# jluuser/PyTorch-VAE

Hardware: AMD Instinct MI355X
Metric: train images/sec @64x64x3 bs256 (curve tensors [B,64,6], SURVEY.md s0) (higher is better)
Workload: dtype f32; 1 GPU; C2: stage2_vq.yaml model with num_quantizers=1 K=512 D=64 N=64; full train step (fwd+loss+bwd+clip+AdamW+EMA), dropout 0.1, loss weights at epoch 100; per_gpu_batch=256, global_batch=256, seq_len=64, parallelism=dp1, hipgraph=True, params=43115078

## Files before the change

### pytorch-vae_amd/csrc/gemm.hip

```cpp
#include "common.h"
#include <type_traits>
#include <utility>
#include <vector>
#include <algorithm>

namespace {

constexpr int BM = 128, BN = 128;
constexpr int BK = 32;
template <int BKT> struct Tile {
    static constexpr int KC_LD = BKT + 4;
    static constexpr int A_TILE = BM * KC_LD;
    static constexpr int NLD = BKT / 8;
};

enum EpiMode {
    EPI_LINEAR = 0,
    EPI_RELU_DROP = 1,
    EPI_GELU = 2,
    EPI_DROP_RESID = 3,
    EPI_SIGMOID = 4,
    EPI_MUL_POSMASK = 5,
    EPI_MUL_GELUGRAD = 6,
    EPI_MUL_SIGGRAD = 7,
// ... 600 lines not shown
    for (int i = threadIdx.x; i < M * nq; i += 256) {
        f32x4 v = *reinterpret_cast<const f32x4*>(red + (size_t)i * 4);
        for (int s2 = 1; s2 < slices; ++s2) v += *reinterpret_cast<const f32x4*>(red + (size_t)s2 * M * N + (size_t)i * 4);
        *reinterpret_cast<f32x4*>(out + (size_t)i * 4) = v;
    }
    if (rs && threadIdx.x < M) {
        float t = 0.f;
        for (int s2 = 0; s2 < slices; ++s2) t += red_rs[s2][threadIdx.x];
        rs[(size_t)blockIdx.x * M + threadIdx.x] = t;
    }
}

#include "gemm_dma.inc"
#include "gemm_p3.inc"

struct ProfRec { int slot; double flops; hipEvent_t e0, e1; };
bool g_prof_on = false;
std::vector<ProfRec> g_prof;
constexpr int PROF_MODES = 9;
constexpr int PROF_FAMILIES = 7;
inline int prof_slot(bool a_kc, bool b_kc, int mode_t, int family = 0) {
    return (family * 4 + (a_kc ? 2 : 0) + (b_kc ? 1 : 0)) * PROF_MODES + mode_t + 1;
}

template <bool A_KC, bool B_KC, int BKT, int MODE = -1>
int launch(const GemmArgs& g, int splits, hipStream_t stream) {
    static bool attr_set = false;
    const size_t smem = (size_t)4 * Tile<BKT>::A_TILE * sizeof(float);
    if (!attr_set) {
        hipError_t e = hipFuncSetAttribute(reinterpret_cast<const void*>(&gemm_f32_mfma<A_KC, B_KC, BKT, MODE>),
// ... 89 lines not shown
            rc = VQH_ERR_LAUNCH;
        } else if (out) {
            out[r.slot * 3 + 0] += 1.0;
            out[r.slot * 3 + 1] += (double)ms * 1e-3;
            out[r.slot * 3 + 2] += r.flops;
        }
        (void)hipEventDestroy(r.e0);
        (void)hipEventDestroy(r.e1);
    }
    g_prof.clear();
    return rc;
}

extern "C" int vqh_reduce_slabs(const float* slabs, int S, long long stride, long long n, float* out, float beta,
                                hipStream_t stream);

static int g_gemm_flags = 1;
extern "C" int vqh_gemm_set_flags(int flags) {
#ifndef VQH_DIAG
    flags &= ~(2 | 4);
#endif
    const int old = g_gemm_flags; g_gemm_flags = flags; return old;
}

static int gemm_impl(int a_kcontig, int b_kcontig, int M, int N, int K, const float* A, int lda, const float* B,
                     int ldb, float* C, int ldc, const float* bias, int mode, const float* aux_in, float* aux_out,
                     int ldaux, float beta, const unsigned long long* rng_state, unsigned drop_site, float drop_p,
                     float* workspace, long long workspace_floats, float* rowsum, hipStream_t stream) {
    VQH_CHECK_ARG(M >= 0 && N >= 0 && K >= 0, "vqh_gemm: negative dimension");
    if (M == 0 || N == 0) return VQH_OK;
// ... 195 lines not shown
extern "C" int vqh_gemm_wgrad(int rows, int n_out, int k_in, const float* dY, int lddy, const float* X, int ldx, float* dW,
                              int lddw, float* db, float beta, float* workspace, long long workspace_floats,
                              hipStream_t stream) {
    if (rows > 0 && n_out > 0 && k_in == 0) return VQH_OK;
    return gemm_impl(0, 0, n_out, k_in, rows, dY, lddy, X, ldx, dW, lddw, nullptr, EPI_LINEAR, nullptr, nullptr, 0, beta,
                     nullptr, 0, 0.f, workspace, workspace_floats, db, stream);
}

struct vqh_wgrad_t {
    int rows, n_out, k_in;
    const float* dY; int lddy;
    const float* X; int ldx;
    float* dW; int lddw;
    float* db;
};
extern "C" int vqh_gemm_wgrad_group(int n, const vqh_wgrad_t* pr, float* workspace, long long workspace_floats,
                                    hipStream_t stream) {
    VQH_CHECK_ARG(n >= 0 && (n == 0 || pr), "vqh_gemm_wgrad_group: bad argument");
    auto al16 = [](const void* q) { return (reinterpret_cast<uintptr_t>(q) & 15) == 0; };
    std::vector<int> big;
    for (int i = 0; i < n; ++i) {
        const vqh_wgrad_t& w = pr[i];
        VQH_CHECK_ARG(w.rows >= 0 && w.n_out >= 0 && w.k_in >= 0, "vqh_gemm_wgrad_group: negative dimension");
        const bool ok = !(g_gemm_flags & (128 | 256)) && workspace && w.rows >= 8 * dma::TBK && (w.rows % dma::TBK) == 0 &&
                        (w.n_out % dma::TBM) == 0 && (w.k_in % dma::TBN) == 0 && w.n_out > 0 && w.k_in > 0 && al16(w.dY) &&
                        al16(w.X) && al16(w.dW) && al16(workspace) && (w.lddy & 3) == 0 && (w.ldx & 3) == 0 && (w.lddw & 3) == 0 &&
                        w.lddy >= w.n_out && w.ldx >= w.k_in && w.lddw >= w.k_in;
        if (ok) {
            big.push_back(i);
        } else {
            const int rc = vqh_gemm_wgrad(w.rows, w.n_out, w.k_in, w.dY, w.lddy, w.X, w.ldx, w.dW, w.lddw, w.db, 0.f, workspace,
                                          workspace_floats, stream);
            if (rc != VQH_OK) return rc;
        }
    }
    for (size_t c0 = 0; c0 < big.size(); c0 += GROUP_MAX) {
        const int m = (int)std::min<size_t>(GROUP_MAX, big.size() - c0);
        long long tiles_tot = 0;
        int kmax = 0;
        for (int j = 0; j < m; ++j) {
            const vqh_wgrad_t& w = pr[big[c0 + j]];
            tiles_tot += (long long)(w.n_out / dma::TBM) * (w.k_in / dma::TBN);
            kmax = std::max(kmax, w.rows);
        }
        int best_kc = kmax;
        double best = -1.0;
        for (int sp = 1; sp <= 64; ++sp) {
            const int kc = ((kmax + sp - 1) / sp + dma::TBK - 1) / dma::TBK * dma::TBK;
            if (kc < 16 * dma::TBK && sp > 1) break;
            long long wgs = 0, slab = 0;
            for (int j = 0; j < m; ++j) {
                const vqh_wgrad_t& w = pr[big[c0 + j]];
                const int splits = (w.rows + kc - 1) / kc;
                wgs += (long long)(w.n_out / dma::TBM) * (w.k_in / dma::TBN) * splits;
                if (splits > 1) slab += (long long)splits * ((long long)w.n_out * w.k_in + w.n_out);
            }
            if (slab > workspace_floats) continue;
            const double rounds = (double)((wgs + 255) / 256);
// ... 27 lines not shown
                off += (long long)splits * w.n_out * w.k_in;
                g.rowsum_ws = w.db ? workspace + off : nullptr;
                if (w.db) off += (long long)splits * w.n_out;
                off = (off + 3) / 4 * 4;
                red[nred++] = Red{g.ws, splits, w.n_out, w.k_in, w.dW, w.lddw, g.rowsum_ws, w.db};
            } else {
                g.ws = nullptr;
                g.rowsum_ws = nullptr;
            }
            G.tiles[j] = (w.n_out / dma::TBM) * (w.k_in / dma::TBN);
            G.wg_begin[j] = wg;
            wg += G.tiles[j] * splits;
            flops += 2.0 * w.n_out * (double)w.k_in * w.rows;
        }
        for (int j = m; j <= GROUP_MAX; ++j) G.wg_begin[j] = wg;
        static bool attr_set = false;
        if (!attr_set) {
            hipError_t e = hipFuncSetAttribute(reinterpret_cast<const void*>(&gemm_f32_dma_group),
                                               hipFuncAttributeMaxDynamicSharedMemorySize, dma::LDS_BYTES);
            if (e == hipSuccess)
                e = hipFuncSetAttribute(reinterpret_cast<const void*>(&gemm_f32_x3_group), hipFuncAttributeMaxDynamicSharedMemorySize,
                                        dma::LDS_BYTES);
            if (e != hipSuccess) { vqh_set_error(hipGetErrorString(e)); return VQH_ERR_LAUNCH; }
            attr_set = true;
        }
        const bool native = (g_gemm_flags & 512) != 0;
        ProfRec rec{};
        if (g_prof_on) {
            rec.slot = prof_slot(false, false, EPI_LINEAR, native ? 2 : 4);
            rec.flops = flops;
            if (hipEventCreate(&rec.e0) != hipSuccess || hipEventCreate(&rec.e1) != hipSuccess ||
                hipEventRecord(rec.e0, stream) != hipSuccess) {
                vqh_set_error("vqh_gemm_wgrad_group: profiling events failed");
                return VQH_ERR_LAUNCH;
            }
        }
        if (native) hipLaunchKernelGGL(gemm_f32_dma_group, dim3(wg), dim3(256), dma::LDS_BYTES, stream, G);
        else hipLaunchKernelGGL(gemm_f32_x3_group, dim3(wg), dim3(256), dma::LDS_BYTES, stream, G);
        VQH_LAUNCH_CHECK();
        if (g_prof_on) {
            if (hipEventRecord(rec.e1, stream) != hipSuccess) {
// ... 55 lines not shown
            VQH_CHECK_ARG(it.X && it.P && it.rows > 0 && it.cols > 0 && (it.cols % 32) == 0 && it.ldx >= it.cols && (it.ldx & 3) == 0 &&
                          it.pitch_bytes >= (long long)it.cols * 6 && (it.pitch_bytes % 16) == 0 &&
                          ((reinterpret_cast<uintptr_t>(it.X) | reinterpret_cast<uintptr_t>(it.P)) & 15) == 0,
                          "vqh_p3_split_multi: bad item (cols % 32, alignment, pitch)");
            S.it[i] = P3SplitItem{it.X, reinterpret_cast<char*>(it.P), it.rows, it.cols, it.ldx, it.pitch_bytes};
            most = std::max(most, (long long)it.rows * (it.cols >> 3));
        }
        int bx = (int)std::min<long long>((most + 255) / 256, 512);
        hipLaunchKernelGGL(p3_split_multi_kernel, dim3(bx, S.n), dim3(256), 0, stream, S);
        VQH_LAUNCH_CHECK();
    }
    return VQH_OK;
}

namespace {
inline int p3_num_cus() {
    static int n = 0;
    if (n == 0) {
        int dev = 0;
        hipDeviceProp_t prop;
        if (hipGetDevice(&dev) == hipSuccess && hipGetDeviceProperties(&prop, dev) == hipSuccess && prop.multiProcessorCount > 0)
            n = prop.multiProcessorCount;
        else n = 256;
    }
    return n;
}
template <bool A_KC, bool B_KC, int MODE>
int launch_p3(const P3Args& g, int splits, hipStream_t stream) {
    static bool attr_set = false;
    auto kern = &gemm_p3<A_KC, B_KC, MODE>;
    if (!attr_set) {
        hipError_t e = hipFuncSetAttribute(reinterpret_cast<const void*>(kern), hipFuncAttributeMaxDynamicSharedMemorySize, p3::LDS_BYTES);
        if (e != hipSuccess) { vqh_set_error(hipGetErrorString(e)); return VQH_ERR_LAUNCH; }
        attr_set = true;
    }
    const int n_items = (g.M / p3::TBM) * (g.N / p3::TBN) * splits;
    dim3 grid(std::min(n_items, p3_num_cus()));
    if (((g.kchunk / p3::TBK) & 1) && n_items > (int)grid.x) grid.x = n_items;
    ProfRec rec{};
    if (g_prof_on) {
        rec.slot = prof_slot(A_KC, B_KC, MODE, 5);
// ... 275 lines not shown
```

### pytorch-vae_amd/csrc/gemm_dma.inc

```

namespace dma {
constexpr int TBM = 256, TBN = 128, TBK = 32;
constexpr int A_BYTES = TBM * TBK * 4, B_BYTES = TBN * TBK * 4, STAGE_BYTES = A_BYTES + B_BYTES;
constexpr int NSTAGE = 3, LDS_BYTES = NSTAGE * STAGE_BYTES;
constexpr int DMA_A = A_BYTES / 1024 / 4, DMA_B = B_BYTES / 1024 / 4, DMA_PER_WAVE = DMA_A + DMA_B;
constexpr int MI = 4, NJ = 2;
}

typedef float f32x2 __attribute__((ext_vector_type(2)));

typedef unsigned u32x2 __attribute__((ext_vector_type(2)));
typedef unsigned u32x4 __attribute__((ext_vector_type(4)));
typedef short s16x4 __attribute__((ext_vector_type(4)));
typedef __bf16 bf16x8 __attribute__((ext_vector_type(8)));

namespace x3 {
constexpr int A_PLANE = dma::TBM * dma::TBK * 2, B_PLANE = dma::TBN * dma::TBK * 2;
constexpr int B_OFF = 3 * A_PLANE;
constexpr int STAGE_BYTES = 3 * (A_PLANE + B_PLANE);
constexpr int LDS_BYTES = 2 * STAGE_BYTES;
constexpr int NU = 12, NUA = 8;
constexpr int NB = 8, G = 48, NSLOT = 96;
constexpr int BAR = 7 * NU;
constexpr int RS_OFF = 40960;
// ... 34 lines not shown
    __device__ __forceinline__ void all(const f32x4& a) { step<0>(a); step<1>(a); step<2>(a); step<3>(a); step<4>(a); }
};

__device__ __forceinline__ void glds16_s(const char* ubase, unsigned voff, unsigned lds_byte_addr_uniform) {
    asm volatile("s_mov_b32 m0, %2\n\ts_nop 0\n\tglobal_load_lds_dwordx4 %0, %1"
                 :
                 : "v"(voff), "s"(ubase), "s"(lds_byte_addr_uniform)
                 : "memory");
}

__device__ __forceinline__ void glds16(const float* gptr, unsigned lds_byte_addr_uniform) {
    __builtin_amdgcn_global_load_lds(gptr, (__attribute__((address_space(3))) void*)(uintptr_t)lds_byte_addr_uniform, 16, 0, 0);
}

template <bool A_KC, bool B_KC, int MODE, bool X3 = false>
__device__ __forceinline__ void gemm_dma_tile(const GemmArgs& g, const int tile, const int zsplit) {
    using namespace dma;
    constexpr bool EA_KC = X3 ? true : A_KC, EB_KC = X3 ? true : B_KC;
    extern __shared__ __attribute__((aligned(1024))) unsigned char smem_dma[];
    const int tid = threadIdx.x, lane = tid & 63;
    const int wave = __builtin_amdgcn_readfirstlane(tid >> 6);
    const int wm = wave >> 1, wn = wave & 1;
    const int l31 = lane & 31, h = lane >> 5;

    const int tiles_n = g.N / TBN;
    const int m0 = (tile / tiles_n) * TBM, n0 = (tile % tiles_n) * TBN;
    const int kbeg = zsplit * g.kchunk;
    const int kend = min(g.K, kbeg + g.kchunk);
    const int nk = (kend - kbeg) / TBK;

    unsigned voff[DMA_PER_WAVE];
    unsigned dst[DMA_PER_WAVE];
#pragma unroll
    for (int i = 0; i < DMA_A; ++i) {
        const int j = wave + 4 * i;
        if (A_KC) {
            const int R = j * 8 + (lane >> 3), c = (lane & 7) ^ ((R >> 1) & 7);
            voff[i] = (unsigned)(((size_t)R * g.lda + c * 4) * 4);
        } else {
            voff[i] = (unsigned)(((size_t)j * g.lda + lane * 4) * 4);
        }
        dst[i] = j * 1024;
    }
// ... 215 lines not shown
                return *reinterpret_cast<const u32x4*>(sb + x3::B_OFF + pl * x3::B_PLANE + j * 2048 + rB[gg]);
            } else {
                const unsigned a0 = (unsigned)(uintptr_t)(sb + x3::B_OFF + pl * x3::B_PLANE + (16 * gg) * 256 + rB[j]);
                const s16x4 lo = __builtin_amdgcn_ds_read_tr16_b64_v4i16((__attribute__((address_space(3))) s16x4*)(uintptr_t)a0);
                const s16x4 hi = __builtin_amdgcn_ds_read_tr16_b64_v4i16((__attribute__((address_space(3))) s16x4*)(uintptr_t)(a0 + 4 * 256));
                const u32x2 l2 = __builtin_bit_cast(u32x2, lo), h2 = __builtin_bit_cast(u32x2, hi);
                return u32x4{l2[0], l2[1], h2[0], h2[1]};
            }
        };
        auto aux_one = [&](auto q_c) {
            constexpr int q = decltype(q_c)::value;
            auxr[q] = *reinterpret_cast<const f32x4*>(g.aux_in + (size_t)(m0 + wm * 128 + (lane >> 4) + q * 4) * g.ldaux + col);
        };
        if (nk > 0) {
            static_for<x3::NU>([&](auto u_c) { load_unit(u_c, 0); });
            if (HAS_DROP && g.drop.p > 0.f && !g.ws) {
#pragma unroll
                for (int qi = 0; qi < 32; ++qi) hash_quad(qi);
            }
            static_for<x3::NU>([&](auto u_c) {
                constexpr int u = decltype(u_c)::value;
                if (do_rowsum && u < x3::NUA) {
#pragma unroll
                    for (int e = 0; e < 4; ++e) rs[e] += st[u][e];
                }
                su.all(st[u]);
                write_unit(u_c, I0{}, smem_dma);
                write_unit(u_c, I1{}, smem_dma);
                write_unit(u_c, I2{}, smem_dma);
                load_unit(u_c, nk > 1 ? 1 : 0);
            });
            asm volatile("s_waitcnt lgkmcnt(0)" ::: "memory");
            __builtin_amdgcn_s_barrier();
            static_for<4>([&](auto i_c) { xA[0][decltype(i_c)::value] = read_A(I0{}, i_c, I0{}, smem_dma); });
            static_for<6>([&](auto x_c) {
                constexpr int x = decltype(x_c)::value;
                xB[0][x / 2][x % 2] = read_B(std::integral_constant<int, x / 2>{}, std::integral_constant<int, x % 2>{}, I0{}, smem_dma);
            });
            auto kstep = [&](auto last_c, const int kt) {
                constexpr bool LAST = decltype(last_c)::value;
                const unsigned char* rstg = smem_dma + (kt & 1) * x3::STAGE_BYTES;
                unsigned char* wstg = smem_dma + ((kt & 1) ^ 1) * x3::STAGE_BYTES;
                const int kt_ld = min(kt + 2, nk - 1);
                const bool want_aux = LAST && HAS_AUX && !g.ws;
                static_for<x3::NSLOT>([&](auto m_c) {
                    constexpr int m = decltype(m_c)::value;
                    constexpr int gg = m / x3::G, mm = m % x3::G, pi = mm / x3::NB, b = mm % x3::NB, i = b / 2, j = b % 2;
                    constexpr int pa = (pi < 3) ? 0 : (pi < 5) ? 1 : 2;
                    constexpr int pb = (pi == 0 || pi == 3 || pi == 5) ? 0 : (pi == 1 || pi == 4) ? 1 : 2;
                    acc[i][j] = __builtin_amdgcn_mfma_f32_32x32x16_bf16(__builtin_bit_cast(bf16x8, xA[pa][i]),
                                                                        __builtin_bit_cast(bf16x8, xB[gg][pb][j]), acc[i][j], 0, 0, 0);
                    if constexpr (m < 8 && m % 2 == 0) xA[1][m / 2] = read_A(I1{}, std::integral_constant<int, m / 2>{}, I0{}, rstg);
                    if constexpr (m >= 8 && m < 16 && m % 2 == 0) xA[2][(m - 8) / 2] = read_A(I2{}, std::integral_constant<int, (m - 8) / 2>{}, I0{}, rstg);
                    if constexpr (m >= 16 && m < 28 && m % 2 == 0) {
                        constexpr int x = (m - 16) / 2;
                        xB[1][x / 2][x % 2] = read_B(std::integral_constant<int, x / 2>{}, std::integral_constant<int, x % 2>{}, I1{}, rstg);
                    }
                    if constexpr (m >= 28 && m < 44 && m % 4 == 0) xA[0][(m - 28) / 4] = read_A(I0{}, std::integral_constant<int, (m - 28) / 4>{}, I1{}, rstg);
                    if constexpr (m >= 48 && m < 56 && m % 2 == 0) xA[1][(m - 48) / 2] = read_A(I1{}, std::integral_constant<int, (m - 48) / 2>{}, I1{}, rstg);
// ... 24 lines not shown
                        if constexpr (m == x3::BAR - 1) {
                            asm volatile("s_waitcnt lgkmcnt(0)" ::: "memory");
                            __builtin_amdgcn_s_barrier();
                        }
                    } else if constexpr (HAS_AUX) {
                        if constexpr (m % 3 == 0) {
                            if (want_aux) aux_one(std::integral_constant<int, m / 3>{});
                        }
                    }
                    __builtin_amdgcn_sched_barrier(0);
                });
            };
            for (int kt = 0; kt < nk - 1; ++kt) kstep(std::false_type{}, kt);
            kstep(std::true_type{}, nk - 1);
            __builtin_amdgcn_s_barrier();
        } else if (HAS_AUX && !g.ws) {
            load_aux_all();
        }
    } else
    if (nk > 0) {
        issue_all(0, 0);
        issue_all(nk > 1 ? 1 : 0, 1);
        if (HAS_DROP && g.drop.p > 0.f && !g.ws) {
#pragma unroll
            for (int qi = 0; qi < 32; ++qi) hash_quad(qi);
        }
        asm volatile("s_waitcnt vmcnt(%0)" ::"n"(DMA_PER_WAVE) : "memory");
        __builtin_amdgcn_s_barrier();
        read_first(0);
        int stage = 0;
        for (int kt = 0; kt < nk; ++kt) {
            const int nxt = (stage == 2) ? 0 : stage + 1;
            const int nx2 = (nxt == 2) ? 0 : nxt + 1;
            if (HAS_AUX && !g.ws && kt == nk - 1) load_aux_all();
            substep(I0{}, I1{}, I0{}, I0{}, stage, 0, 0);
            substep(I1{}, I2{}, I0{}, I0{}, stage, 0, 0);
            asm volatile("s_waitcnt vmcnt(0)" ::: "memory");
            __builtin_amdgcn_s_barrier();
            const int ktd = min(kt + 2, nk - 1);
            substep(I0{}, I3{}, I0{}, IH{}, stage, ktd, nx2);
            substep(I1{}, I0{}, IH{}, IF{}, nxt, ktd, nx2);
            stage = nxt;
        }
        asm volatile("s_waitcnt vmcnt(0)" ::: "memory");
        __builtin_amdgcn_s_barrier();
    } else if (HAS_AUX && !g.ws) {
        load_aux_all();
    }

    if (X3 && do_rowsum) {
        float* rsb = reinterpret_cast<float*>(smem_dma + x3::RS_OFF);
        *reinterpret_cast<f32x4*>(rsb + wave * TBM + 4 * lane) = f32x4{rs[0], rs[1], rs[2], rs[3]};
        __builtin_amdgcn_s_barrier();
        if (wave == 0) {
            f32x4 t = *reinterpret_cast<const f32x4*>(rsb + 4 * lane);
#pragma unroll
            for (int w = 1; w < 4; ++w) t += *reinterpret_cast<const f32x4*>(rsb + w * TBM + 4 * lane);
            const int row = m0 + 4 * lane;
            if (g.rowsum_ws) {
                *reinterpret_cast<f32x4*>(g.rowsum_ws + (size_t)zsplit * g.M + row) = t;
            } else {
#pragma unroll
                for (int i = 0; i < 4; ++i) g.rowsum[row + i] = (g.beta != 0.f) ? g.beta * g.rowsum[row + i] + t[i] : t[i];
            }
        }
    } else
    if (do_rowsum) {
#pragma unroll
        for (int i = 0; i < 4; ++i) rs[i] += __shfl_xor(rs[i], 32, 64);
        if (h == 0) {
            const int row = m0 + wm * 128 + 4 * l31;
            if (g.rowsum_ws) {
                *reinterpret_cast<f32x4*>(g.rowsum_ws + (size_t)zsplit * g.M + row) = f32x4{rs[0], rs[1], rs[2], rs[3]};
            } else {
#pragma unroll
                for (int i = 0; i < 4; ++i)
                    g.rowsum[row + i] = (g.beta != 0.f) ? g.beta * g.rowsum[row + i] + rs[i] : rs[i];
            }
        }
    }

    const int mode = (MODE >= 0) ? MODE : g.mode;
    constexpr int EP_LD = 68;
    float* ep = reinterpret_cast<float*>(smem_dma) + wave * (32 * EP_LD);
    float* slab = g.ws ? g.ws + (size_t)zsplit * g.M * g.N : nullptr;
    if constexpr (X3 && MODE == EPI_LINEAR) {
        if (!(g.flags & 2048)) {
            const size_t ldo = slab ? (size_t)g.N : (size_t)g.ldc;
            float* obase = slab ? slab : g.C;
#pragma unroll
            for (int j = 0; j < NJ; ++j) {
                const int cj = n0 + wn * 64 + j * 32 + l31;
                const float bj = (g.bias && !slab) ? g.bias[cj] : 0.f;
                float* cp = obase + (size_t)(m0 + wm * 128 + 4 * h) * ldo + cj;
                if (!slab && g.beta != 0.f) {
#pragma unroll
                    for (int i = 0; i < MI; ++i)
#pragma unroll
                        for (int r = 0; r < 16; ++r) {
                            float* q = cp + (size_t)(i * 32 + (r & 3) + 8 * (r >> 2)) * ldo;
// ... 74 lines not shown
                } else if (mode == EPI_MUL_GELUGRAD) {
#pragma unroll
                    for (int e = 0; e < 4; ++e) v[e] *= gelu_erf_grad(a[e]);
                } else {
#pragma unroll
                    for (int e = 0; e < 4; ++e) v[e] *= a[e] * (1.f - a[e]);
                }
            }
            if (g.beta != 0.f) v += g.beta * *reinterpret_cast<const f32x4*>(cptr);
            *reinterpret_cast<f32x4*>(cptr) = v;
        }
        __builtin_amdgcn_s_waitcnt(0xC07F);
    }
}

template <bool A_KC, bool B_KC, int MODE>
__global__ __launch_bounds__(256, 1) void gemm_f32_dma(const GemmArgs g) {
    const int nx = gridDim.x, nt = nx * gridDim.z, lin = blockIdx.z * nx + blockIdx.x;
    const int q = nt >> 3, r = nt & 7, x = lin & 7, j = lin >> 3;
    const int v = (x < r ? x * (q + 1) : r * (q + 1) + (x - r) * q) + j;
    gemm_dma_tile<A_KC, B_KC, MODE>(g, v % nx, v / nx);
}

template <bool A_KC, bool B_KC, int MODE>
__global__ __launch_bounds__(256, 1) void gemm_f32_x3(const GemmArgs g) {
    const int nx = gridDim.x, nt = nx * gridDim.z, lin = blockIdx.z * nx + blockIdx.x;
    const int q = nt >> 3, r = nt & 7, x = lin & 7, j = lin >> 3;
    const int v = (x < r ? x * (q + 1) : r * (q + 1) + (x - r) * q) + j;
    gemm_dma_tile<A_KC, B_KC, MODE, true>(g, v % nx, v / nx);
}
// ... 16 lines not shown
    const int v = ((G.p[0].flags & 1) && !(G.p[0].flags & 1024)) ? group_logical_id() : (int)blockIdx.x;
    int p = 0;
    while (p + 1 < G.n && v >= G.wg_begin[p + 1]) ++p;
    const int local = v - G.wg_begin[p];
    const int tiles = G.tiles[p];
    gemm_dma_tile<false, false, EPI_LINEAR>(G.p[p], local % tiles, local / tiles);
}
__global__ __launch_bounds__(256, 1) void gemm_f32_x3_group(const GemmGroupArgs G) {
    const int v = ((G.p[0].flags & 1) && !(G.p[0].flags & 1024)) ? group_logical_id() : (int)blockIdx.x;
    int p = 0;
    while (p + 1 < G.n && v >= G.wg_begin[p + 1]) ++p;
    const int local = v - G.wg_begin[p];
    const int tiles = G.tiles[p];
    gemm_dma_tile<false, false, EPI_LINEAR, true>(G.p[p], local % tiles, local / tiles);
}
```

### pytorch-vae_amd/csrc/loss.hip

```cpp
#include "common.h"

namespace {

enum { T_VALID = 0, T_PAIR = 1, T_TRI = 2, T_QUAD = 3, T_FIVE = 4, T_ANY3 = 5, T_PDM = 8, T_LR = 40 };

enum {
    P_RAW = 0, P_ALN, P_BEST, P_RMSD_RAW, P_RMSD_BEST, P_CE, P_ACC, P_SSTV, P_BL, P_BA, P_DIR, P_DIH, P_TV2, P_TAU,
    P_PDM, P_LRPDM, P_WINK, P_COMMIT, P_KAPPA, P_COUNT
};

enum {
    M_LOSS = 0, M_REC_XYZ, M_MSE_RAW, M_MSE_ALN, M_REC_SS, M_SS_ACC, M_VQ_LOSS, M_BL, M_BA, M_DIR, M_DIH, M_GEOM,
    M_SS_TV, M_USAGE_REG, M_TV2, M_PPL, M_DEAD, M_RMSD_RAW, M_RMSD_ALN, M_PDM, M_WINK, M_KAPPA, M_TAU, M_LRPDM, M_COUNT
};

struct LossCfg {
    int B, L, Ntok, D;
    int Ls;
    const float* Ldev;
    int masked;
    int use_vq;
    float rmsd_w, ss_w, bl_w, ba_w, dir_w, dih_w, tv_l, pdm_w, wk_w, kap_w, tau_w, lr_w;
    float alpha, ss_tv_l, label_smoothing, beta;
    int pdm_window, wk_size, wk_stride, lr_sep, lr_stride, lr_max;
// ... 205 lines not shown
        double R[9];
        kabsch_rotation(Hm, R);
        bool ok = true;
        for (int k = 0; k < 9; ++k) { Rt_s[k] = (float)R[k]; ok = ok && isfinite(R[k]); }
        for (int j = 0; j < 3; ++j) {
            const double t = bmu[j] - (amu[0] * R[0 * 3 + j] + amu[1] * R[1 * 3 + j] + amu[2] * R[2 * 3 + j]);
            Rt_s[9 + j] = (float)t;
            ok = ok && isfinite(t);
        }
        Rt_s[12] = ok ? 1.f : 0.f;
    }
    __syncthreads();
    return Rt_s[12] != 0.f;
}

__global__ __launch_bounds__(256) void loss_counts_kernel(const unsigned char* __restrict__ mask, LossCfg c_in,
                                                          int* __restrict__ table) {
    const LossCfg c = loss_resolve(c_in);
    extern __shared__ unsigned char sm_[];
    unsigned char* m = sm_;
    const int b = blockIdx.x, L = c.L;
    for (int l = threadIdx.x; l < L; l += 256) m[l] = mask ? mask[(size_t)b * c.Ls + l] : 1;
    __syncthreads();
    int nv = 0, np = 0, nt = 0, nq = 0, n5 = 0;
    for (int l = threadIdx.x; l < L; l += 256) {
        nv += m[l];
        if (l + 1 < L) np += m[l] & m[l + 1];
        if (l + 2 < L) nt += m[l] & m[l + 1] & m[l + 2];
        if (l + 3 < L) nq += m[l] & m[l + 1] & m[l + 2] & m[l + 3];
        if (l + 4 < L) n5 += m[l] & m[l + 1] & m[l + 2] & m[l + 3] & m[l + 4];
    }
    __shared__ int red[5];
    if (threadIdx.x < 5) red[threadIdx.x] = 0;
    __syncthreads();
    atomicAdd(&red[0], nv); atomicAdd(&red[1], np); atomicAdd(&red[2], nt); atomicAdd(&red[3], nq); atomicAdd(&red[4], n5);
    __syncthreads();
    if (threadIdx.x == 0) {
        atomicAdd(&table[T_VALID], red[0]); atomicAdd(&table[T_PAIR], red[1]); atomicAdd(&table[T_TRI], red[2]);
        atomicAdd(&table[T_QUAD], red[3]); atomicAdd(&table[T_FIVE], red[4]);
        if (red[0] >= 3) atomicAdd(&table[T_ANY3], 1);
    }
    for (int d = 1 + (threadIdx.x >> 6); d < c.pdm_window && d < 32; d += 4) {
        int s = 0;
        for (int l = threadIdx.x & 63; l + d < L; l += 64) s += m[l] & m[l + d];
        for (int o = 32; o > 0; o >>= 1) s += __shfl_xor(s, o, 64);
        if ((threadIdx.x & 63) == 0 && s) atomicAdd(&table[T_PDM + d - 1], s);
    }
    {
        int p = 0;
        for (int off = 0; off < max(1, c.lr_max); ++off)
            for (int i = 0; i < L; i += max(1, c.lr_stride)) {
                const int j = i + c.lr_sep + off;
                if (j >= L) break;
                if ((p & 255) == (int)threadIdx.x && (m[i] & m[j])) atomicAdd(&table[T_LR + p], 1);
                ++p;
            }
    }
    for (int w = threadIdx.x; w < c.n_windows; w += 256) {
        const int s0 = w * max(1, c.wk_stride);
        int cnt = 0;
        for (int l = 0; l < c.wk_size; ++l) cnt += m[s0 + l];
        if (!c.masked || cnt >= 3) atomicAdd(&table[c.t_wk + w], 1);
    }
}

#define FOR_POS(n_) for (int base_ = 0; base_ < (n_); base_ += 256)

__global__ __launch_bounds__(256) void loss_sample_kernel(const float* __restrict__ recons,
                                                          const float* __restrict__ target,
                                                          const unsigned char* __restrict__ mask,
                                                          const float* __restrict__ ze, const float* __restrict__ zq,
                                                          const int* __restrict__ table, LossCfg c_in,
                                                          float* __restrict__ d_recons, float* __restrict__ d_ze,
                                                          float* __restrict__ part) {
    extern __shared__ __attribute__((aligned(16))) float sm[];
    const LossCfg c = loss_resolve(c_in);
    const int L = c.L, b = blockIdx.x, tid = threadIdx.x;
    double* dred = reinterpret_cast<double*>(sm);
// ... 461 lines not shown
    for (int k = 0; k < 3; ++k) { c.sd[k] = data_stats ? data_stats[k] : 1.f; c.mu[k] = data_stats ? data_stats[3 + k] : 0.f; }
    VQH_CHECK_ARG(c.pdm_window <= 33, "vqh_loss_fwd_bwd: pdm_window > 33 unsupported");
    int npairs = 0, nwin = 0;
    loss_enumerate(L_dev ? L_stride : L, c.lr_sep, c.lr_stride, c.lr_max, c.wk_size, c.wk_stride, &npairs, &nwin);
    c.n_lr_pairs = npairs;
    c.n_windows = nwin;
    c.t_wk = T_LR + npairs;
    const long long table_ints = c.t_wk + nwin + 8;
    const long long need = table_ints + (long long)B * P_COUNT;
    VQH_CHECK_ARG(need <= workspace_floats, "vqh_loss_fwd_bwd: workspace too small");
    int* table = reinterpret_cast<int*>(workspace);
    float* part = workspace + table_ints;
    hipError_t e = hipMemsetAsync(table, 0, sizeof(int) * table_ints, stream);
    if (e != hipSuccess) { vqh_set_error(hipGetErrorString(e)); return VQH_ERR_LAUNCH; }
    const int Lmax = c.L;
    hipLaunchKernelGGL(loss_counts_kernel, dim3(B), dim3(256), (size_t)Lmax, stream, mask, c, table);
    const size_t smem = sizeof(float) * (size_t)(8 + 23 * Lmax + 4 + 16 + 9 * Lmax + 4);
    VQH_CHECK_ARG(smem <= 160 * 1024, "vqh_loss_fwd_bwd: sequence too long for the LDS-resident loss kernel");
    static bool attr_set = false;
    if (!attr_set) {
        hipError_t ea = hipFuncSetAttribute(reinterpret_cast<const void*>(&loss_sample_kernel),
                                            hipFuncAttributeMaxDynamicSharedMemorySize, 160 * 1024);
        if (ea != hipSuccess) { vqh_set_error(hipGetErrorString(ea)); return VQH_ERR_LAUNCH; }
        attr_set = true;
    }
    hipLaunchKernelGGL(loss_sample_kernel, dim3(B), dim3(256), smem, stream, recons, target, mask, ze, zq, table, c,
                       d_recons, d_ze, part);
    hipLaunchKernelGGL(loss_finish_kernel, dim3(1), dim3(64), 0, stream, part, table, c, vq_stats, metrics);
    VQH_LAUNCH_CHECK();
    return VQH_OK;
}
// ... 1 lines not shown
```

Before: 9684 images/s.

## Balance grouped wgrad GEMM via stream-K ranges and batch loss count kernel

```diff
diff --git a/pytorch-vae_amd/csrc/gemm.hip b/pytorch-vae_amd/csrc/gemm.hip
--- a/pytorch-vae_amd/csrc/gemm.hip
+++ b/pytorch-vae_amd/csrc/gemm.hip
@@ -638,6 +638,49 @@
 #include "gemm_dma.inc"
 #include "gemm_p3.inc"
 
+struct RedRangeArgs {
+    GroupRangePlan P;
+    struct Item { const float* ws; int M, N; float* C; int ldc; const float* rs_ws; float* rowsum; } r[GROUP_MAX];
+};
+__global__ __launch_bounds__(256) void splitk_reduce_ranges(const RedRangeArgs G) {
+    const GroupRangePlan& P = G.P;
+    const int gt = blockIdx.y;
+    int p = 0;
+    while (p + 1 < P.n && gt >= P.tbeg[p + 1]) ++p;
+    const int tile = gt - P.tbeg[p], nk = P.nk[p];
+    const int t0 = P.sbeg[p] + tile * nk, t1 = t0 + nk;
+    int v = min(P.wgs - 1, (int)(((long long)t0 * P.wgs) / P.total));
+    while (range_bound(P, v + 1) <= t0) ++v;
+    while (range_bound(P, v) > t0) --v;
+    int cnt = 1;
+    while (range_bound(P, v + cnt) < t1) ++cnt;
+    if (cnt == 1) return;
+    const RedRangeArgs::Item& it = G.r[p];
+    const int tiles_n = it.N / dma::TBN;
+    const int m0 = (tile / tiles_n) * dma::TBM, n0 = (tile % tiles_n) * dma::TBN;
+    const int tid = threadIdx.x;
+    if (it.rowsum && n0 == 0 && blockIdx.x == 0) {
+        float s = 0.f;
+        for (int z = 0; z < cnt; ++z) s += it.rs_ws[(size_t)z * it.M + m0 + tid];
+        it.rowsum[m0 + tid] = s;
+    }
+    const size_t total = (size_t)it.M * it.N;
+    const int row0 = m0 + 64 * blockIdx.x + (tid >> 5), col = n0 + (tid & 31) * 4;
+    const float* src = it.ws + (size_t)row0 * it.N + col;
+    f32x4 s[8];
+#pragma unroll
+    for (int i = 0; i < 8; ++i) s[i] = f32x4{0.f, 0.f, 0.f, 0.f};
+    for (int z = 0; z < cnt; ++z) {
+        f32x4 x[8];
+#pragma unroll
+        for (int i = 0; i < 8; ++i) x[i] = *reinterpret_cast<const f32x4*>(src + (size_t)z * total + (size_t)(8 * i) * it.N);
+#pragma unroll
+        for (int i = 0; i < 8; ++i) s[i] += x[i];
+    }
+#pragma unroll
+    for (int i = 0; i < 8; ++i) *reinterpret_cast<f32x4*>(it.C + (size_t)(row0 + 8 * i) * it.ldc + col) = s[i];
+}
+
 struct ProfRec { int slot; double flops; hipEvent_t e0, e1; };
 bool g_prof_on = false;
 std::vector<ProfRec> g_prof;
@@ -757,6 +800,18 @@
 
 extern "C" int vqh_reduce_slabs(const float* slabs, int S, long long stride, long long n, float* out, float beta,
                                 hipStream_t stream);
+
+static int gemm_num_cus() {
+    static int n = 0;
+    if (n == 0) {
+        int dev = 0;
+        hipDeviceProp_t prop;
+        if (hipGetDevice(&dev) == hipSuccess && hipGetDeviceProperties(&prop, dev) == hipSuccess && prop.multiProcessorCount > 0)
+            n = prop.multiProcessorCount;
+        else n = 256;
+    }
+    return n;
+}
 
 static int g_gemm_flags = 1;
 extern "C" int vqh_gemm_set_flags(int flags) {
@@ -982,6 +1037,95 @@
     float* dW; int lddw;
     float* db;
 };
+constexpr int VQH_DEFER = -1000;
+static int wgrad_group_ranges(int m, const vqh_wgrad_t* pr, const int* sel, float* workspace, long long workspace_floats,
+                              bool native, hipStream_t stream) {
+    GroupRangePlan P;
+    P.n = m; P.wgs = gemm_num_cus(); P.snap = 2;
+    long long tot = 0;
+    int tiles_tot = 0;
+    for (int j = 0; j < m; ++j) {
+        const vqh_wgrad_t& w = pr[sel[j]];
+        const int tiles = (w.n_out / dma::TBM) * (w.k_in / dma::TBN);
+        P.nk[j] = w.rows / dma::TBK;
+        P.sbeg[j] = (int)tot; P.tbeg[j] = tiles_tot;
+        tot += (long long)tiles * P.nk[j];
+        tiles_tot += tiles;
+        if (tot >= (1LL << 30) || tiles_tot > 65535) return VQH_DEFER;
+    }
+    for (int j = m; j <= GROUP_MAX; ++j) { P.sbeg[j] = (int)tot; P.tbeg[j] = tiles_tot; }
+    for (int j = m; j < GROUP_MAX; ++j) P.nk[j] = 1;
+    P.total = (int)tot; P.q = P.total / P.wgs; P.r = P.total % P.wgs;
+    if (P.q < 16 || P.wgs > 32768) return VQH_DEFER;
+    std::vector<int> cuts(tiles_tot, 0);
+    for (int v = 1; v < P.wgs; ++v) {
+        const int b = range_bound(P, v), p = range_problem(P, b), local = b - P.sbeg[p];
+        if (local % P.nk[p]) ++cuts[P.tbeg[p] + local / P.nk[p]];
+    }
+    GemmGroupArgs G;
+    RedRangeArgs RG;
+    G.n = m;
+    RG.P = P;
+    long long off = 0;
+    double flops = 0.0;
+    bool any = false;
+    for (int j = 0; j < m; ++j) {
+        const vqh_wgrad_t& w = pr[sel[j]];
+        int slabs = 1;
+        for (int t = P.tbeg[j]; t < P.tbeg[j + 1]; ++t) slabs = std::max(slabs, 1 + cuts[t]);
+        GemmArgs& g = G.p[j];
+        g.A = w.dY; g.B = w.X; g.C = w.dW;
+        g.M = w.n_out; g.N = w.k_in; g.K = w.rows;
+        g.lda = w.lddy; g.ldb = w.ldx; g.ldc = w.lddw;
+        g.kchunk = w.rows;
+        g.vecA = g.vecB = g.vecC = 1;
+        g.mode = EPI_LINEAR; g.bias = nullptr; g.aux_in = nullptr; g.aux_out = nullptr; g.ldaux = 0; g.beta = 0.f;
+        g.drop = make_drop(nullptr, 0, 0.f);
+        g.flags = g_gemm_flags;
+        g.rowsum = w.db;
+        g.ws = nullptr; g.rowsum_ws = nullptr;
+        if (slabs > 1) {
+            g.ws = workspace + off;
+            off += (long long)slabs * w.n_out * w.k_in;
+            if (w.db) { g.rowsum_ws = workspace + off; off += (long long)slabs * w.n_out; }
+            off = (off + 3) / 4 * 4;
+            any = true;
+        }
+        RG.r[j] = RedRangeArgs::Item{g.ws, w.n_out, w.k_in, w.dW, w.lddw, g.rowsum_ws, w.db};
+        G.tiles[j] = P.tbeg[j + 1] - P.tbeg[j];
+        G.wg_begin[j] = 0;
+        flops += 2.0 * w.n_out * (double)w.k_in * w.rows;
+    }
+    for (int j = m; j <= GROUP_MAX; ++j) G.wg_begin[j] = 0;
+    for (int j = m; j < GROUP_MAX; ++j) { G.tiles[j] = 0; RG.r[j] = RedRangeArgs::Item{nullptr, 0, 0, nullptr, 0, nullptr, nullptr}; }
+    if (off > workspace_floats) return VQH_DEFER;
+    ProfRec rec{};
+    if (g_prof_on) {
+        rec.slot = prof_slot(false, false, EPI_LINEAR, native ? 2 : 4);
+        rec.flops = flops;
+        if (hipEventCreate(&rec.e0) != hipSuccess || hipEventCreate(&rec.e1) != hipSuccess ||
+            hipEventRecord(rec.e0, stream) != hipSuccess) {
+            vqh_set_error("vqh_gemm_wgrad_group: profiling events failed");
+            return VQH_ERR_LAUNCH;
+        }
+    }
+    if (native) hipLaunchKernelGGL(gemm_f32_dma_group_ranges, dim3(P.wgs), dim3(256), dma::LDS_BYTES, stream, G, P);
+    else hipLaunchKernelGGL(gemm_f32_x3_group_ranges, dim3(P.wgs), dim3(256), dma::LDS_BYTES, stream, G, P);
+    VQH_LAUNCH_CHECK();
+    if (g_prof_on) {
+        if (hipEventRecord(rec.e1, stream) != hipSuccess) {
+            vqh_set_error("vqh_gemm_wgrad_group: profiling events failed");
+            return VQH_ERR_LAUNCH;
+        }
+        g_prof.push_back(rec);
+    }
+    if (any) {
+        hipLaunchKernelGGL(splitk_reduce_ranges, dim3(4, tiles_tot), dim3(256), 0, stream, RG);
+        VQH_LAUNCH_CHECK();
+    }
+    return VQH_OK;
+}
+
 extern "C" int vqh_gemm_wgrad_group(int n, const vqh_wgrad_t* pr, float* workspace, long long workspace_floats,
                                     hipStream_t stream) {
     VQH_CHECK_ARG(n >= 0 && (n == 0 || pr), "vqh_gemm_wgrad_group: bad argument");
@@ -1004,12 +1148,25 @@
     }
     for (size_t c0 = 0; c0 < big.size(); c0 += GROUP_MAX) {
         const int m = (int)std::min<size_t>(GROUP_MAX, big.size() - c0);
-        long long tiles_tot = 0;
         int kmax = 0;
-        for (int j = 0; j < m; ++j) {
-            const vqh_wgrad_t& w = pr[big[c0 + j]];
-            tiles_tot += (long long)(w.n_out / dma::TBM) * (w.k_in / dma::TBN);
-            kmax = std::max(kmax, w.rows);
+        for (int j = 0; j < m; ++j) kmax = std::max(kmax, pr[big[c0 + j]].rows);
+        static bool attr_set = false;
+        if (!attr_set) {
+            for (const void* f : {reinterpret_cast<const void*>(&gemm_f32_dma_group), reinterpret_cast<const void*>(&gemm_f32_x3_group),
+                                  reinterpret_cast<const void*>(&gemm_f32_dma_group_ranges),
+                                  reinterpret_cast<const void*>(&gemm_f32_x3_group_ranges)}) {
+                const hipError_t e = hipFuncSetAttribute(f, hipFuncAttributeMaxDynamicSharedMemorySize, dma::LDS_BYTES);
+                if (e != hipSuccess) { vqh_set_error(hipGetErrorString(e)); return VQH_ERR_LAUNCH; }
+            }
+            attr_set = true;
+        }
+        const bool native = (g_gemm_flags & 512) != 0;
+        if (!(g_gemm_flags & 4096)) {
+            const int rc = wgrad_group_ranges(m, pr, &big[c0], workspace, workspace_floats, native, stream);
+            if (rc != VQH_DEFER) {
+                if (rc != VQH_OK) return rc;
+                continue;
+            }
         }
         int best_kc = kmax;
         double best = -1.0;
@@ -1067,17 +1224,6 @@
             flops += 2.0 * w.n_out * (double)w.k_in * w.rows;
         }
         for (int j = m; j <= GROUP_MAX; ++j) G.wg_begin[j] = wg;
-        static bool attr_set = false;
-        if (!attr_set) {
-            hipError_t e = hipFuncSetAttribute(reinterpret_cast<const void*>(&gemm_f32_dma_group),
-                                               hipFuncAttributeMaxDynamicSharedMemorySize, dma::LDS_BYTES);
-            if (e == hipSuccess)
-                e = hipFuncSetAttribute(reinterpret_cast<const void*>(&gemm_f32_x3_group), hipFuncAttributeMaxDynamicSharedMemorySize,
-                                        dma::LDS_BYTES);
-            if (e != hipSuccess) { vqh_set_error(hipGetErrorString(e)); return VQH_ERR_LAUNCH; }
-            attr_set = true;
-        }
-        const bool native = (g_gemm_flags & 512) != 0;
         ProfRec rec{};
         if (g_prof_on) {
             rec.slot = prof_slot(false, false, EPI_LINEAR, native ? 2 : 4);
@@ -1163,17 +1309,7 @@
 }
 
 namespace {
-inline int p3_num_cus() {
-    static int n = 0;
-    if (n == 0) {
-        int dev = 0;
-        hipDeviceProp_t prop;
-        if (hipGetDevice(&dev) == hipSuccess && hipGetDeviceProperties(&prop, dev) == hipSuccess && prop.multiProcessorCount > 0)
-            n = prop.multiProcessorCount;
-        else n = 256;
-    }
-    return n;
-}
+inline int p3_num_cus() { return gemm_num_cus(); }
 template <bool A_KC, bool B_KC, int MODE>
 int launch_p3(const P3Args& g, int splits, hipStream_t stream) {
     static bool attr_set = false;
diff --git a/pytorch-vae_amd/csrc/gemm_dma.inc b/pytorch-vae_amd/csrc/gemm_dma.inc
--- a/pytorch-vae_amd/csrc/gemm_dma.inc
+++ b/pytorch-vae_amd/csrc/gemm_dma.inc
@@ -72,7 +72,8 @@
 }
 
 template <bool A_KC, bool B_KC, int MODE, bool X3 = false>
-__device__ __forceinline__ void gemm_dma_tile(const GemmArgs& g, const int tile, const int zsplit) {
+__device__ __forceinline__ void gemm_dma_tile_k(const GemmArgs& g, const int tile, const int kbeg, const int kend,
+                                                float* const slab, float* const rs_slab) {
     using namespace dma;
     constexpr bool EA_KC = X3 ? true : A_KC, EB_KC = X3 ? true : B_KC;
     extern __shared__ __attribute__((aligned(1024))) unsigned char smem_dma[];
@@ -83,8 +84,6 @@
 
     const int tiles_n = g.N / TBN;
     const int m0 = (tile / tiles_n) * TBM, n0 = (tile % tiles_n) * TBN;
-    const int kbeg = zsplit * g.kchunk;
-    const int kend = min(g.K, kbeg + g.kchunk);
     const int nk = (kend - kbeg) / TBK;
 
     unsigned voff[DMA_PER_WAVE];
@@ -330,7 +329,7 @@
         };
         if (nk > 0) {
             static_for<x3::NU>([&](auto u_c) { load_unit(u_c, 0); });
-            if (HAS_DROP && g.drop.p > 0.f && !g.ws) {
+            if (HAS_DROP && g.drop.p > 0.f && !slab) {
 #pragma unroll
                 for (int qi = 0; qi < 32; ++qi) hash_quad(qi);
             }
@@ -358,7 +357,7 @@
                 const unsigned char* rstg = smem_dma + (kt & 1) * x3::STAGE_BYTES;
                 unsigned char* wstg = smem_dma + ((kt & 1) ^ 1) * x3::STAGE_BYTES;
                 const int kt_ld = min(kt + 2, nk - 1);
-                const bool want_aux = LAST && HAS_AUX && !g.ws;
+                const bool want_aux = LAST && HAS_AUX && !slab;
                 static_for<x3::NSLOT>([&](auto m_c) {
                     constexpr int m = decltype(m_c)::value;
                     constexpr int gg = m / x3::G, mm = m % x3::G, pi = mm / x3::NB, b = mm % x3::NB, i = b / 2, j = b % 2;
@@ -413,14 +412,14 @@
             for (int kt = 0; kt < nk - 1; ++kt) kstep(std::false_type{}, kt);
             kstep(std::true_type{}, nk - 1);
             __builtin_amdgcn_s_barrier();
-        } else if (HAS_AUX && !g.ws) {
+        } else if (HAS_AUX && !slab) {
             load_aux_all();
         }
     } else
     if (nk > 0) {
         issue_all(0, 0);
         issue_all(nk > 1 ? 1 : 0, 1);
-        if (HAS_DROP && g.drop.p > 0.f && !g.ws) {
+        if (HAS_DROP && g.drop.p > 0.f && !slab) {
 #pragma unroll
             for (int qi = 0; qi < 32; ++qi) hash_quad(qi);
         }
@@ -431,7 +430,7 @@
         for (int kt = 0; kt < nk; ++kt) {
             const int nxt = (stage == 2) ? 0 : stage + 1;
             const int nx2 = (nxt == 2) ? 0 : nxt + 1;
-            if (HAS_AUX && !g.ws && kt == nk - 1) load_aux_all();
+            if (HAS_AUX && !slab && kt == nk - 1) load_aux_all();
             substep(I0{}, I1{}, I0{}, I0{}, stage, 0, 0);
             substep(I1{}, I2{}, I0{}, I0{}, stage, 0, 0);
             asm volatile("s_waitcnt vmcnt(0)" ::: "memory");
@@ -443,7 +442,7 @@
         }
         asm volatile("s_waitcnt vmcnt(0)" ::: "memory");
         __builtin_amdgcn_s_barrier();
-    } else if (HAS_AUX && !g.ws) {
+    } else if (HAS_AUX && !slab) {
         load_aux_all();
     }
 
@@ -456,8 +455,8 @@
 #pragma unroll
             for (int w = 1; w < 4; ++w) t += *reinterpret_cast<const f32x4*>(rsb + w * TBM + 4 * lane);
             const int row = m0 + 4 * lane;
-            if (g.rowsum_ws) {
-                *reinterpret_cast<f32x4*>(g.rowsum_ws + (size_t)zsplit * g.M + row) = t;
+            if (rs_slab) {
+                *reinterpret_cast<f32x4*>(rs_slab + row) = t;
             } else {
 #pragma unroll
                 for (int i = 0; i < 4; ++i) g.rowsum[row + i] = (g.beta != 0.f) ? g.beta * g.rowsum[row + i] + t[i] : t[i];
@@ -469,8 +468,8 @@
         for (int i = 0; i < 4; ++i) rs[i] += __shfl_xor(rs[i], 32, 64);
         if (h == 0) {
             const int row = m0 + wm * 128 + 4 * l31;
-            if (g.rowsum_ws) {
-                *reinterpret_cast<f32x4*>(g.rowsum_ws + (size_t)zsplit * g.M + row) = f32x4{rs[0], rs[1], rs[2], rs[3]};
+            if (rs_slab) {
+                *reinterpret_cast<f32x4*>(rs_slab + row) = f32x4{rs[0], rs[1], rs[2], rs[3]};
             } else {
 #pragma unroll
                 for (int i = 0; i < 4; ++i)
@@ -482,7 +481,6 @@
     const int mode = (MODE >= 0) ? MODE : g.mode;
     constexpr int EP_LD = 68;
     float* ep = reinterpret_cast<float*>(smem_dma) + wave * (32 * EP_LD);
-    float* slab = g.ws ? g.ws + (size_t)zsplit * g.M * g.N : nullptr;
     if constexpr (X3 && MODE == EPI_LINEAR) {
         if (!(g.flags & 2048)) {
             const size_t ldo = slab ? (size_t)g.N : (size_t)g.ldc;
@@ -587,6 +585,14 @@
     }
 }
 
+template <bool A_KC, bool B_KC, int MODE, bool X3 = false>
+__device__ __forceinline__ void gemm_dma_tile(const GemmArgs& g, const int tile, const int zsplit) {
+    const int kbeg = zsplit * g.kchunk;
+    gemm_dma_tile_k<A_KC, B_KC, MODE, X3>(g, tile, kbeg, min(g.K, kbeg + g.kchunk),
+                                          g.ws ? g.ws + (size_t)zsplit * g.M * g.N : nullptr,
+                                          g.rowsum_ws ? g.rowsum_ws + (size_t)zsplit * g.M : nullptr);
+}
+
 template <bool A_KC, bool B_KC, int MODE>
 __global__ __launch_bounds__(256, 1) void gemm_f32_dma(const GemmArgs g) {
     const int nx = gridDim.x, nt = nx * gridDim.z, lin = blockIdx.z * nx + blockIdx.x;
@@ -633,3 +639,58 @@
     const int tiles = G.tiles[p];
     gemm_dma_tile<false, false, EPI_LINEAR, true>(G.p[p], local % tiles, local / tiles);
 }
+
+struct GroupRangePlan {
+    int n, wgs, snap;
+    int total, q, r;
+    int sbeg[GROUP_MAX + 1];
+    int tbeg[GROUP_MAX + 1];
+    int nk[GROUP_MAX];
+};
+__host__ __device__ inline int range_problem(const GroupRangePlan& P, const int t) {
+    int p = 0;
+    while (p + 1 < P.n && t >= P.sbeg[p + 1]) ++p;
+    return p;
+}
+__host__ __device__ inline int range_bound(const GroupRangePlan& P, const int v) {
+    if (v <= 0) return 0;
+    if (v >= P.wgs) return P.total;
+    const int raw = v * P.q + (v * P.r) / P.wgs;
+    const int p = range_problem(P, raw);
+    const int k = (raw - P.sbeg[p]) % P.nk[p];
+    if (k < P.snap) return raw - k;
+    if (P.nk[p] - k < P.snap) return raw + (P.nk[p] - k);
+    return raw;
+}
+
+template <bool X3>
+__device__ __forceinline__ void gemm_group_ranges(const GemmGroupArgs& G, const GroupRangePlan& P) {
+    const int v = ((G.p[0].flags & 1) && !(G.p[0].flags & 1024)) ? group_logical_id() : (int)blockIdx.x;
+    int t = range_bound(P, v);
+    const int e = range_bound(P, v + 1);
+    while (t < e) {
+        const int p = range_problem(P, t);
+        const int nk = P.nk[p];
+        const int local = t - P.sbeg[p], tile = local / nk, k0 = local - tile * nk;
+        const int k1 = min(nk, k0 + (e - t));
+        const GemmArgs& g = G.p[p];
+        float *slab = nullptr, *rs_slab = nullptr;
+        if (k0 != 0 || k1 != nk) {
+            const int t0 = t - k0;
+            int idx = 0;
+            for (int vv = v; range_bound(P, vv) > t0; --vv) ++idx;
+            slab = g.ws + (size_t)idx * g.M * g.N;
+            rs_slab = g.rowsum_ws ? g.rowsum_ws + (size_t)idx * g.M : nullptr;
+        }
+        gemm_dma_tile_k<false, false, EPI_LINEAR, X3>(g, tile, k0 * dma::TBK, k1 * dma::TBK, slab, rs_slab);
+        t += k1 - k0;
+        asm volatile("s_waitcnt lgkmcnt(0)" ::: "memory");
+        __builtin_amdgcn_s_barrier();
+    }
+}
+__global__ __launch_bounds__(256, 1) void gemm_f32_dma_group_ranges(const GemmGroupArgs G, const GroupRangePlan P) {
+    gemm_group_ranges<false>(G, P);
+}
+__global__ __launch_bounds__(256, 1) void gemm_f32_x3_group_ranges(const GemmGroupArgs G, const GroupRangePlan P) {
+    gemm_group_ranges<true>(G, P);
+}
diff --git a/pytorch-vae_amd/csrc/loss.hip b/pytorch-vae_amd/csrc/loss.hip
--- a/pytorch-vae_amd/csrc/loss.hip
+++ b/pytorch-vae_amd/csrc/loss.hip
@@ -243,54 +243,67 @@
     return Rt_s[12] != 0.f;
 }
 
+constexpr int COUNTS_SAMPLES_PER_BLOCK = 16;
 __global__ __launch_bounds__(256) void loss_counts_kernel(const unsigned char* __restrict__ mask, LossCfg c_in,
-                                                          int* __restrict__ table) {
+                                                          int* __restrict__ table, int table_ints) {
     const LossCfg c = loss_resolve(c_in);
-    extern __shared__ unsigned char sm_[];
-    unsigned char* m = sm_;
-    const int b = blockIdx.x, L = c.L;
-    for (int l = threadIdx.x; l < L; l += 256) m[l] = mask ? mask[(size_t)b * c.Ls + l] : 1;
-    __syncthreads();
-    int nv = 0, np = 0, nt = 0, nq = 0, n5 = 0;
-    for (int l = threadIdx.x; l < L; l += 256) {
-        nv += m[l];
-        if (l + 1 < L) np += m[l] & m[l + 1];
-        if (l + 2 < L) nt += m[l] & m[l + 1] & m[l + 2];
-        if (l + 3 < L) nq += m[l] & m[l + 1] & m[l + 2] & m[l + 3];
-        if (l + 4 < L) n5 += m[l] & m[l + 1] & m[l + 2] & m[l + 3] & m[l + 4];
-    }
-    __shared__ int red[5];
-    if (threadIdx.x < 5) red[threadIdx.x] = 0;
-    __syncthreads();
-    atomicAdd(&red[0], nv); atomicAdd(&red[1], np); atomicAdd(&red[2], nt); atomicAdd(&red[3], nq); atomicAdd(&red[4], n5);
-    __syncthreads();
-    if (threadIdx.x == 0) {
-        atomicAdd(&table[T_VALID], red[0]); atomicAdd(&table[T_PAIR], red[1]); atomicAdd(&table[T_TRI], red[2]);
-        atomicAdd(&table[T_QUAD], red[3]); atomicAdd(&table[T_FIVE], red[4]);
-        if (red[0] >= 3) atomicAdd(&table[T_ANY3], 1);
-    }
-    for (int d = 1 + (threadIdx.x >> 6); d < c.pdm_window && d < 32; d += 4) {
-        int s = 0;
-        for (int l = threadIdx.x & 63; l + d < L; l += 64) s += m[l] & m[l + d];
-        for (int o = 32; o > 0; o >>= 1) s += __shfl_xor(s, o, 64);
-        if ((threadIdx.x & 63) == 0 && s) atomicAdd(&table[T_PDM + d - 1], s);
-    }
-    {
-        int p = 0;
-        for (int off = 0; off < max(1, c.lr_max); ++off)
-            for (int i = 0; i < L; i += max(1, c.lr_stride)) {
-                const int j = i + c.lr_sep + off;
-                if (j >= L) break;
-                if ((p & 255) == (int)threadIdx.x && (m[i] & m[j])) atomicAdd(&table[T_LR + p], 1);
-                ++p;
-            }
-    }
-    for (int w = threadIdx.x; w < c.n_windows; w += 256) {
-        const int s0 = w * max(1, c.wk_stride);
-        int cnt = 0;
-        for (int l = 0; l < c.wk_size; ++l) cnt += m[s0 + l];
-        if (!c.masked || cnt >= 3) atomicAdd(&table[c.t_wk + w], 1);
-    }
+    extern __shared__ __attribute__((aligned(16))) unsigned char sm_[];
+    int* tab = reinterpret_cast<int*>(sm_);
+    unsigned char* m = sm_ + sizeof(int) * (size_t)table_ints;
+    __shared__ int nv_s;
+    const int L = c.L, tid = threadIdx.x, lane = tid & 63;
+    for (int k = tid; k < table_ints; k += 256) tab[k] = 0;
+    for (int b = blockIdx.x; b < c.B; b += gridDim.x) {
+        if (tid == 0) nv_s = 0;
+        __syncthreads();
+        for (int l = tid; l < L; l += 256) m[l] = mask ? mask[(size_t)b * c.Ls + l] : 1;
+        __syncthreads();
+        int n[5] = {0, 0, 0, 0, 0};
+        for (int l = tid; l < L; l += 256) {
+            n[0] += m[l];
+            if (l + 1 < L) n[1] += m[l] & m[l + 1];
+            if (l + 2 < L) n[2] += m[l] & m[l + 1] & m[l + 2];
+            if (l + 3 < L) n[3] += m[l] & m[l + 1] & m[l + 2] & m[l + 3];
+            if (l + 4 < L) n[4] += m[l] & m[l + 1] & m[l + 2] & m[l + 3] & m[l + 4];
+        }
+#pragma unroll
+        for (int k = 0; k < 5; ++k) {
+            for (int o = 32; o > 0; o >>= 1) n[k] += __shfl_xor(n[k], o, 64);
+            if (lane == 0 && n[k]) atomicAdd(&tab[T_VALID + k], n[k]);
+        }
+        if (lane == 0 && n[0]) atomicAdd(&nv_s, n[0]);
+        for (int d = 1 + (tid >> 6); d < c.pdm_window && d < 32; d += 4) {
+            int s = 0;
+            for (int l = lane; l + d < L; l += 64) s += m[l] & m[l + d];
+            for (int o = 32; o > 0; o >>= 1) s += __shfl_xor(s, o, 64);
+            if (lane == 0 && s) atomicAdd(&tab[T_PDM + d - 1], s);
+        }
+        {
+            const int st = max(1, c.lr_stride);
+            int p0 = 0;
+            for (int off = 0; off < max(1, c.lr_max); ++off) {
+                const int span = min(L, L - c.lr_sep - off);
+                if (span <= 0) continue;
+                const int np = (span + st - 1) / st;
+                for (int q = tid; q < np; q += 256) {
+                    const int i = q * st;
+                    if (m[i] & m[i + c.lr_sep + off]) atomicAdd(&tab[T_LR + p0 + q], 1);
+                }
+                p0 += np;
+            }
+        }
+        for (int w = tid; w < c.n_windows; w += 256) {
+            const int s0 = w * max(1, c.wk_stride);
+            int cnt = 0;
+            for (int l = 0; l < c.wk_size; ++l) cnt += m[s0 + l];
+            if (!c.masked || cnt >= 3) atomicAdd(&tab[c.t_wk + w], 1);
+        }
+        __syncthreads();
+        if (tid == 0 && nv_s >= 3) tab[T_ANY3] += 1;
+    }
+    __syncthreads();
+    for (int k = tid; k < table_ints; k += 256)
+        if (tab[k]) atomicAdd(&table[k], tab[k]);
 }
 
 #define FOR_POS(n_) for (int base_ = 0; base_ < (n_); base_ += 256)
@@ -782,7 +795,9 @@
     hipError_t e = hipMemsetAsync(table, 0, sizeof(int) * table_ints, stream);
     if (e != hipSuccess) { vqh_set_error(hipGetErrorString(e)); return VQH_ERR_LAUNCH; }
     const int Lmax = c.L;
-    hipLaunchKernelGGL(loss_counts_kernel, dim3(B), dim3(256), (size_t)Lmax, stream, mask, c, table);
+    VQH_CHECK_ARG(sizeof(int) * (size_t)table_ints + (size_t)Lmax <= 64 * 1024, "vqh_loss_fwd_bwd: count table too large for LDS");
+    hipLaunchKernelGGL(loss_counts_kernel, dim3((B + COUNTS_SAMPLES_PER_BLOCK - 1) / COUNTS_SAMPLES_PER_BLOCK), dim3(256),
+                       sizeof(int) * (size_t)table_ints + (size_t)Lmax, stream, mask, c, (int*)table, (int)table_ints);
     const size_t smem = sizeof(float) * (size_t)(8 + 23 * Lmax + 4 + 16 + 9 * Lmax + 4);
     VQH_CHECK_ARG(smem <= 160 * 1024, "vqh_loss_fwd_bwd: sequence too long for the LDS-resident loss kernel");
     static bool attr_set = false;
```

Result: no change. 9683 images/s (-0.0%).
